# DJATOM/x265-aMod

Measured on AMD Instinct MI355X. Metric: encoded frames/sec at 1080p & 2160p --preset medium; bit-exact vs CPU ref, higher is better.
Workload: dtype u8

## Files before the change

include/x265amd.h:

```cpp
#ifndef X265AMD_H
#define X265AMD_H

#include <stdint.h>
#include <stddef.h>

#ifdef __cplusplus
extern "C" {
#endif

#ifndef X265AMD_DEPTH
#define X265AMD_DEPTH 8
#endif
#if X265AMD_DEPTH > 8
typedef uint16_t x265amd_pixel;
#else
typedef uint8_t x265amd_pixel;
#endif

#define X265AMD_OK 0
#define X265AMD_EINVAL (-1)
#define X265AMD_EHIP (-2)
#define X265AMD_ENOMEM (-3)

int x265amd_bit_depth(void);
// ... 349 lines not shown
    int32_t stride[3];
    int32_t bitDepth;
    int32_t layout;
    int32_t clipMin, clipMax;
    int32_t reserved;
} x265amd_surface;
#endif
int x265amd_ingest_picture(void* stream, const x265amd_surface* d_src, int srcW, int srcH,
                           x265amd_pixel* d_pic , int W, int H, int marginX, int marginY);
int x265amd_ingest_model(const x265amd_surface* src, int srcW, int srcH, x265amd_pixel* pic, int W, int H, int marginX, int marginY);

#define X265AMD_DB_INTRA 1
#define X265AMD_DB_CBF 2
#define X265AMD_DB_BYPASS 4
#define X265AMD_DB_TU_LEFT 8
#define X265AMD_DB_PU_LEFT 16
#define X265AMD_DB_TU_TOP 32
#define X265AMD_DB_PU_TOP 64
typedef struct x265amd_slice_info x265amd_slice_info;
typedef struct x265amd_mvpred_info x265amd_mvpred_info;
typedef struct x265amd_cu_unit x265amd_cu_unit;
typedef struct x265amd_mv_unit x265amd_mv_unit;
typedef struct x265amd_deblock_unit { uint8_t flags; int8_t qp; int8_t ref[2]; int16_t mv[2][2]; } x265amd_deblock_unit;
int x265amd_deblock_picture(void* stream, x265amd_pixel* d_y, x265amd_pixel* d_u, x265amd_pixel* d_v, intptr_t stride, intptr_t cstride,
                            int width, int height, const x265amd_deblock_unit* d_units, int betaOffsetDiv2, int tcOffsetDiv2,
                            int cbQpOffset, int crQpOffset, int bypassEnabled, int passes);

int x265amd_deblock_rows(void* stream, x265amd_pixel* d_y, x265amd_pixel* d_u, x265amd_pixel* d_v, intptr_t stride, intptr_t cstride,
                         int width, int height, const x265amd_deblock_unit* d_units, int betaOffsetDiv2, int tcOffsetDiv2,
                         int cbQpOffset, int crQpOffset, int bypassEnabled, int passes, int y4_begin, int y4_end);
int x265amd_deblock_rows_cols(void* stream, x265amd_pixel* d_y, x265amd_pixel* d_u, x265amd_pixel* d_v, intptr_t stride, intptr_t cstride,
                              int width, int height, const x265amd_deblock_unit* d_units, int betaOffsetDiv2, int tcOffsetDiv2,
                              int cbQpOffset, int crQpOffset, int bypassEnabled, int passes, int y4_begin, int y4_end, int ctu_col_begin, int ctu_col_end);

int x265amd_deblock_units(const x265amd_slice_info* si, const x265amd_mvpred_info* info, const x265amd_cu_unit* units, const x265amd_mv_unit* motion,
                          x265amd_deblock_unit* out);
int x265amd_deblock_units_rows(const x265amd_slice_info* si, const x265amd_mvpred_info* info, const x265amd_cu_unit* units, const x265amd_mv_unit* motion,
                               x265amd_deblock_unit* out, int y4_begin, int y4_end);
int x265amd_deblock_units_rect(const x265amd_slice_info* si, const x265amd_mvpred_info* info, const x265amd_cu_unit* units, const x265amd_mv_unit* motion,
                               x265amd_deblock_unit* out, int y4_begin, int y4_end, int x4_begin, int x4_end);

typedef struct x265amd_sao_ctu
{
    int8_t type[2];
    uint8_t band_pos[3];
    int8_t offset[3][4];
    uint8_t reserved[3];
} x265amd_sao_ctu;
int x265amd_sao_stats(void* stream, const uint64_t rec_planes[3], const uint64_t fenc_planes[3], intptr_t stride, intptr_t cstride,
                      int width, int height, int32_t* d_count, int32_t* d_offset_org);
int x265amd_sao_apply(void* stream, const uint64_t src_planes[3], const uint64_t dst_planes[3], intptr_t stride, intptr_t cstride,
                      int width, int height, const x265amd_sao_ctu* d_params);
int x265amd_sao_stats_rows(void* stream, const uint64_t rec_planes[3], const uint64_t fenc_planes[3], intptr_t stride, intptr_t cstride,
                           int width, int height, int32_t* d_count, int32_t* d_offset_org, int ctu_row_begin, int ctu_row_end);
int x265amd_sao_apply_rows(void* stream, const uint64_t src_planes[3], const uint64_t dst_planes[3], intptr_t stride, intptr_t cstride,
                           int width, int height, const x265amd_sao_ctu* d_params, int ctu_row_begin, int ctu_row_end);
int x265amd_sao_stats_rows_cols(void* stream, const uint64_t rec_planes[3], const uint64_t fenc_planes[3], intptr_t stride, intptr_t cstride,
                                int width, int height, int32_t* d_count, int32_t* d_offset_org, int ctu_row_begin, int ctu_row_end, int ctu_col_begin, int ctu_col_end);
int x265amd_sao_apply_rows_cols(void* stream, const uint64_t src_planes[3], const uint64_t dst_planes[3], intptr_t stride, intptr_t cstride,
                                int width, int height, const x265amd_sao_ctu* d_params, int ctu_row_begin, int ctu_row_end, int x_begin, int x_end);
enum { X265AMD_SAO_NON_DEBLOCK = 1, X265AMD_SAO_EO01_ONLY = 2 };
int x265amd_sao_stats_opt(void* stream, const uint64_t rec_planes[3], const uint64_t fenc_planes[3], intptr_t stride, intptr_t cstride,
                          int width, int height, int32_t* d_count, int32_t* d_offset_org, int flags);
int x265amd_sao_stats_opt_rows(void* stream, const uint64_t rec_planes[3], const uint64_t fenc_planes[3], intptr_t stride, intptr_t cstride,
                               int width, int height, int32_t* d_count, int32_t* d_offset_org, int flags, int ctu_row_begin, int ctu_row_end);
int x265amd_sao_stats_opt_rows_cols(void* stream, const uint64_t rec_planes[3], const uint64_t fenc_planes[3], intptr_t stride, intptr_t cstride,
                                    int width, int height, int32_t* d_count, int32_t* d_offset_org, int flags, int ctu_row_begin, int ctu_row_end, int ctu_col_begin, int ctu_col_end);
int x265amd_sao_stats_pre(void* stream, const uint64_t rec_planes[3], const uint64_t fenc_planes[3], intptr_t stride, intptr_t cstride,
                          int width, int height, int32_t* d_pre_count, int32_t* d_pre_offset_org);
int x265amd_sao_stats_pre_rows(void* stream, const uint64_t rec_planes[3], const uint64_t fenc_planes[3], intptr_t stride, intptr_t cstride,
                               int width, int height, int32_t* d_pre_count, int32_t* d_pre_offset_org, int ctu_row_begin, int ctu_row_end);
int x265amd_sao_stats_model(const void* const rec_planes[3], const void* const fenc_planes[3], const void* const pre_planes[3], intptr_t stride, intptr_t cstride,
                            int width, int height, int flags, int32_t* pre_count, int32_t* pre_offset_org, int32_t* count, int32_t* offset_org);

enum { X265AMD_FILTER_TOP = 0, X265AMD_FILTER_FULL = 1 };
typedef struct x265amd_filter_step { int32_t kind, row, col_begin, col_end, y4_begin, y4_end, rec_y4_end, rec_x4_begin, rec_x4_end; } x265amd_filter_step;
typedef struct x265amd_filter_finish { int32_t row, x_begin, x_end, y_begin, y_end; } x265amd_filter_finish;
int x265amd_filter_plan(int width, int height, const int32_t* analysed, int32_t* done_top, int32_t* done_full, int32_t* pub_x,
                        int min_chunk, int min_chunk_last, int early_top,
                        x265amd_filter_step* steps, int* num_steps, x265amd_filter_finish* finish, int* num_finish);
int x265amd_filter_ready(int width, int height, const int32_t* analysed, const int32_t* done_top, const int32_t* done_full,
                         int min_chunk, int min_chunk_last, int early_top);

enum { X265AMD_MODE_NONE = 0, X265AMD_MODE_INTER = 1, X265AMD_MODE_INTRA = 2, X265AMD_MODE_SKIP = 3 };
typedef struct x265amd_cu_unit
{
    uint8_t depth;
    uint8_t pred_mode;
    uint8_t part_size;
    uint8_t tu_depth;
    uint8_t luma_dir, chroma_dir;
    uint8_t merge_flag, inter_dir;
    uint8_t cbf[3];
    uint8_t tq_bypass;
    int8_t qp;
    int8_t ref_idx[2];
    uint8_t mvp_idx[2];
    uint8_t reserved;
    int16_t mvd[2][2];
} x265amd_cu_unit;
typedef struct x265amd_slice_info
{
    int32_t pic_width, pic_height;
    int32_t slice_type;
    int32_t slice_qp;
    int32_t num_ref_idx[2];
    int32_t max_num_merge_cand;
    int32_t use_dqp, max_cu_dqp_depth;
    int32_t sign_hide, tq_bypass_enabled;
    int32_t wpp;
    int32_t max_cu_depth;
    int32_t max_amp_depth;
    int32_t tu_log2_min, tu_log2_max;
    int32_t tu_max_depth_inter, tu_max_depth_intra;
} x265amd_slice_info;
#define X265AMD_SLICE_SIGN_HIDE 1
#define X265AMD_SLICE_LOWPASS_DCT 0x100
typedef struct x265amd_cabac x265amd_cabac;
x265amd_cabac* x265amd_cabac_open(const x265amd_slice_info* si, x265amd_cu_unit* units, int bits_only);
void x265amd_cabac_close(x265amd_cabac*);
void x265amd_cabac_set_contexts(x265amd_cabac*, const uint8_t* ctx);
void x265amd_cabac_get_contexts(const x265amd_cabac*, uint8_t* ctx);
int x265amd_cabac_encode_ctu(x265amd_cabac*, int ctu_addr, const int16_t* coeffY, const int16_t* coeffU, const int16_t* coeffV);
uint64_t x265amd_cabac_frac_bits(const x265amd_cabac*);
uint64_t x265amd_cabac_ctu_bits(const x265amd_cabac*);
size_t x265amd_cabac_finish_slice(x265amd_cabac*, uint8_t* out, size_t cap);

typedef struct x265amd_mv_unit { uint8_t pred_mode, inter_dir; int8_t ref_idx[2]; int16_t mv[2][2]; } x265amd_mv_unit;
typedef struct x265amd_mvpred_info
{
    int32_t pic_width, pic_height;
    int32_t is_inter_b, num_ref_idx[2], max_num_merge_cand;
    int32_t temporal_mvp;
    int32_t col_from_l0, check_ldc;
    int32_t poc, ref_poc[2][16];
    int32_t col_poc, col_ref_poc[2][16];
} x265amd_mvpred_info;
typedef struct x265amd_merge_cand { int16_t mv[2][2]; int8_t ref_idx[2]; uint8_t dir; uint8_t reserved; } x265amd_merge_cand;
int x265amd_merge_candidates(const x265amd_mvpred_info* info, const x265amd_mv_unit* cur, const x265amd_mv_unit* col, int cu_x, int cu_y, int log2_cu_size,
                             int part_size, int pu_idx, x265amd_merge_cand* out);
int x265amd_amvp_candidates(const x265amd_mvpred_info* info, const x265amd_mv_unit* cur, const x265amd_mv_unit* col, int cu_x, int cu_y, int log2_cu_size,
                            int part_size, int pu_idx, int list, int ref_idx, int16_t amvp[2][2], int16_t mvc[12][2]);

typedef struct x265amd_inter_search_params
{
    int32_t search_method, subpel_refine, search_range;
    int32_t qp;
    int32_t chroma_mc;
    int32_t ref_pic[2][16];
    int32_t frame_parallel;
    int32_t lazy_sync;
    int32_t lowres_blocks_in_row;
    int32_t me_pic[2][16];
    int32_t weighted;
    x265amd_weight wp[2][16][3];
    uint64_t lowres_mvs[2][16];
} x265amd_inter_search_params;
typedef struct x265amd_inter_cu { int16_t x, y; uint8_t log2_size, part_size; uint8_t reserved[2]; } x265amd_inter_cu;
typedef struct x265amd_pu_result
{
    uint8_t merge_flag, inter_dir;
    int8_t ref_idx[2];
    uint8_t mvp_idx[2];
    uint8_t reserved[2];
    int16_t mv[2][2], mvd[2][2];
} x265amd_pu_result;
// ... 298 lines not shown
```

x265-amod_amd/csrc/encoder_api.hip:

```cpp
#include "encoder_impl.h"
#include "ingest_dev.h"

extern "C" void x265amd_param_default(x265amd_param* p)
{
    if (!p) return;
    memset(p, 0, sizeof(*p));
    p->fpsNum = 25; p->fpsDenom = 1;
    p->bframes = 0; p->keyframeMax = 250; p->maxNumReferences = 3; p->qp = 30; p->ipFactor = 1.4f; p->pbFactor = 1.3f;
    p->rateControlMode = X265AMD_RC_CQP; p->rfConstant = 28; p->aqStrength = 1.0; p->qCompress = 0.6; p->aqMode = 0; p->cuTree = 0; p->qgSize = 32; p->qpMin = 0; p->qpMax = 69; p->vuiVideoFormat = 5; p->vuiColorPrimaries = 2; p->vuiTransfer = 2; p->vuiMatrix = 2; p->bEmitCLL = 1;
    p->rdLevel = 3; p->limitReferences = 3; p->bEnableEarlySkip = 1; p->recursionSkipMode = 1; p->bIntraInBFrames = 1; p->psyRd = 2.0; p->edgeVarThreshold = 0.05f;
    p->searchMethod = X265AMD_ME_HEX; p->subpelRefine = 2; p->searchRange = 57; p->maxNumMergeCand = 3;
    p->bEnableSignHiding = 1; p->bEnableStrongIntraSmoothing = 1; p->bEnableTemporalMvp = 1; p->tuQTMaxInterDepth = 1; p->tuQTMaxIntraDepth = 1;
    p->bEnableLoopFilter = 1; p->bEnableSAO = 1; p->bEnableWavefront = 1; p->aspectRatioIdc = 0;
}

void x265amd_encoder::fillStreamParams(x265amd_stream_params& s) const
{
    memset(&s, 0, sizeof(s));
    static const struct { uint32_t maxLumaSamples, maxLumaSamplesPerSecond; int idc; } levels[] = {
        { 36864, 552960, 30 }, { 122880, 3686400, 60 }, { 245760, 7372800, 63 }, { 552960, 16588800, 90 }, { 983040, 33177600, 93 },
        { 2228224, 66846720, 120 }, { 2228224, 133693440, 123 }, { 8912896, 267386880, 150 }, { 8912896, 534773760, 153 },
        { 8912896, 1069547520, 156 }, { 35651584, 1069547520, 180 }, { 35651584, 2139095040u, 183 }, { 35651584, 4278190080u, 186 } };
    s.profile_idc = X265AMD_DEPTH <= 8 ? 1 : 2;
    s.profile_compatibility_flags = X265AMD_DEPTH <= 8 ? (1u << 1) | (1u << 2) : (1u << 2);
// ... 248 lines not shown
    e->fillStreamParams(sp);
    e->headerBytes.resize(512);
    const size_t n = x265amd_write_stream_headers(&sp, e->headerBytes.data(), e->headerBytes.size());
    if (!n || n > e->headerBytes.size()) { xa_fail(X265AMD_EINVAL, "encoder_open: stream headers"); return nullptr; }
    e->headerBytes.resize(n);
    if (p->bEmitHDR10SEI || p->hasMasteringDisplay || p->maxCLL || p->maxFALL)
    {
        uint8_t sei[64], payload[24];
        if (p->bEmitCLL)
        {
            payload[0] = (uint8_t)(p->maxCLL >> 8); payload[1] = (uint8_t)p->maxCLL; payload[2] = (uint8_t)(p->maxFALL >> 8); payload[3] = (uint8_t)p->maxFALL;
            const size_t m = x265amd_write_sei(0, 144, payload, 4, sei, sizeof(sei));
            if (!m) { xa_fail(X265AMD_EINVAL, "encoder_open: content light level SEI"); return nullptr; }
            e->headerBytes.insert(e->headerBytes.end(), sei, sei + m);
        }
        if (p->hasMasteringDisplay)
        {
            for (int i = 0; i < 8; i++) { payload[2 * i] = (uint8_t)(p->masteringDisplay[i] >> 8); payload[2 * i + 1] = (uint8_t)p->masteringDisplay[i]; }
            for (int i = 0; i < 2; i++)
                for (int k = 0; k < 4; k++) payload[16 + 4 * i + k] = (uint8_t)(p->masteringDisplay[8 + i] >> (24 - 8 * k));
            const size_t m = x265amd_write_sei(0, 137, payload, 24, sei, sizeof(sei));
            if (!m) { xa_fail(X265AMD_EINVAL, "encoder_open: mastering display SEI"); return nullptr; }
            e->headerBytes.insert(e->headerBytes.end(), sei, sei + m);
        }
    }
    if (p->bEmitInfoSEI)
    {
        char text[1024];
        snprintf(text, sizeof(text), "x265amd (x265 build 209 interface) - %s - H.265/HEVC codec on AMD Instinct MI355X - options: %dx%d fps=%u/%u bitdepth=%d %s=%g aq-mode=%d aq-strength=%.2f "
                 "cutree=%d qcomp=%.2f qg-size=%d bframes=%d b-adapt=%d b-pyramid=%d open-gop=%d keyint=%d min-keyint=%d scenecut=%d rc-lookahead=%d lookahead-slices=%d ref=%d limit-refs=%d "
                 "rd=%d rdoq-level=%d psy-rd=%.2f me=%d subme=%d merange=%d max-merge=%d rect=%d amp=%d limit-modes=%d early-skip=%d rskip=%d weightp=%d weightb=%d sao=%d deblock=%d wpp=%d "
                 "tu-intra-depth=%d tu-inter-depth=%d signhide=%d strong-intra-smoothing=%d temporal-mvp=%d b-intra=%d fast-intra=%d sao-non-deblock=%d selective-sao=%d limit-sao=%d",
                 x265amd_version(), p->sourceWidth, p->sourceHeight, p->fpsNum, p->fpsDenom, X265AMD_DEPTH, p->rateControlMode == X265AMD_RC_CRF ? "crf" : "qp",
                 p->rateControlMode == X265AMD_RC_CRF ? p->rfConstant : (double)p->qp, e->aqOn ? p->aqMode : 0, p->aqStrength, p->cuTree != 0, p->qCompress, p->qgSize, p->bframes, p->bFrameAdaptive,
                 p->bBPyramid != 0, p->bOpenGOP != 0, p->keyframeMax, e->keyframeMin, p->scenecutThreshold, p->lookaheadDepth, p->lookaheadSlices, p->maxNumReferences, p->limitReferences,
                 p->rdLevel, p->rdoqLevel, p->psyRd, p->searchMethod, p->subpelRefine, p->searchRange, p->maxNumMergeCand, p->bEnableRectInter != 0, p->bEnableAMP != 0, p->limitModes != 0,
                 p->bEnableEarlySkip != 0, p->recursionSkipMode, p->bEnableWeightedPred != 0, p->bEnableWeightedBiPred != 0, p->bEnableSAO != 0, p->bEnableLoopFilter != 0, p->bEnableWavefront != 0,
                 p->tuQTMaxIntraDepth, p->tuQTMaxInterDepth, p->bEnableSignHiding != 0, p->bEnableStrongIntraSmoothing != 0, p->bEnableTemporalMvp != 0, p->bIntraInBFrames != 0, p->bEnableFastIntra != 0,
                 e->saoNonDeblock, e->selectiveSAO, e->limitSAO);
        if (e->lowPassDct) strncat(text, " lowpass-dct=1", sizeof(text) - strlen(text) - 1);
        uint8_t sei[1400];
        const size_t m = x265amd_write_info_sei(text, sei, sizeof(sei));
        if (!m) { xa_fail(X265AMD_EINVAL, "encoder_open: info SEI"); return nullptr; }
        e->headerBytes.insert(e->headerBytes.end(), sei, sei + m);
    }
    return e.release();
}

static PicP picByCoding(x265amd_encoder* e, uint64_t k)
{
    std::lock_guard<std::mutex> lk(e->byCodingMu);
    auto it = e->byCoding.find(k);
    return it == e->byCoding.end() ? PicP() : it->second;
}
static void rowRanges(const x265amd_encoder& e, int row, uint64_t off[3], uint64_t bytes[3])
{
    for (int k = 0; k < 3; k++)
    {
        const int sh = k ? 1 : 0, my = e.marginY >> sh, mx = e.marginX >> sh, h = e.H >> sh, rowH = 64 >> sh;
        const intptr_t st = k ? e.cstride : e.stride;
        const int y0 = row == 0 ? -my : row * rowH, y1 = row == e.ctuH - 1 ? h + my : std::min(h, (row + 1) * rowH);
        const int64_t first = (int64_t)e.org[k] + (int64_t)y0 * st - mx;
        off[k] = (uint64_t)first * sizeof(pixel);
        bytes[k] = (uint64_t)((int64_t)(y1 - y0) * st) * sizeof(pixel);
    }
}
extern "C" int x265amd_encoder_ctu_rows(const x265amd_encoder* e) { return e ? e->ctuH : -1; }
extern "C" int x265amd_encoder_stats(const x265amd_encoder* e, uint64_t* out, int n)
{
    if (!e || !out || n < 4) return xa_fail(X265AMD_EINVAL, "encoder_stats: arguments"), -1;
    out[0] = e->statPictures[0]; out[1] = e->statPictures[1]; out[2] = e->statPictures[2]; out[3] = e->statReferences;
    if (n >= 13)
        for (int t = 0; t < 3; t++) { out[4 + t] = e->statEmitted[t]; out[7 + t] = e->statBits[t]; memcpy(&out[10 + t], &e->statQpSum[t], 8); }
    if (n >= 31)
    {
        for (int g = 0; g < 4; g++)
        {
            for (int k = 0; k < 3; k++) memcpy(&out[13 + 4 * g + k], &e->statPsnr[g][k], 8);
            memcpy(&out[13 + 4 * g + 3], &e->statSsim[g], 8);
        }
        out[29] = e->statMaxCll;
        memcpy(&out[30], &e->statFallSum, 8);
    }
    return 0;
}
extern "C" int x265amd_encoder_quality(const x265amd_encoder* e, x265amd_quality* out)
{
    if (!e || !out) return xa_fail(X265AMD_EINVAL, "encoder_quality: arguments"), -1;
    if (!e->haveQuality || !e->lastQuality.measured) return -1;
    *out = e->lastQuality;
    return 0;
}
int x265amd_encoder::measureLevel(Pic& pic)
{
    x265amd_luma_level_record level;
    if (x265amd_luma_level(nullptr, planeAddr(pic.dSrc, 0), stride, srcW, srcH, levelDev) != X265AMD_OK) return -1;
    if (hipMemcpy(&level, levelDev, sizeof(level), hipMemcpyDeviceToHost) != hipSuccess) return xa_fail(X265AMD_EHIP, "encoder_encode: light level");
    x265amd_quality_values v;
    if (x265amd_quality_finish(nullptr, nullptr, &level, W, H, srcW, srcH, &v) != X265AMD_OK) return xa_fail(X265AMD_EINVAL, "encoder_encode: light level");
    pic.quality.lumaSum = level.sum; pic.quality.maxLumaLevel = level.max; pic.quality.avgLumaLevel = v.avgLumaLevel; pic.quality.measured |= 4;
    return 0;
}
extern "C" int x265amd_encoder_row_geometry(const x265amd_encoder* e, int row, x265amd_row_export* out)
{
    if (!e || !out || row < 0 || row >= e->ctuH) return xa_fail(X265AMD_EINVAL, "encoder_row_geometry: bad arguments"), -1;
    memset(out, 0, sizeof(*out));
    out->ctu_row = row;
    rowRanges(*e, row, out->plane_offset, out->plane_bytes);
    const size_t u0 = (size_t)row * 16 * e->w4, u1 = (size_t)std::min(e->h4, (row + 1) * 16) * e->w4;
    out->units_bytes = (u1 - u0) * sizeof(x265amd_cu_unit); out->map_offset_units = u0 * sizeof(x265amd_cu_unit);
    out->motion_bytes = (u1 - u0) * sizeof(x265amd_mv_unit); out->map_offset_motion = u0 * sizeof(x265amd_mv_unit);
    return 0;
}
extern "C" int x265amd_encoder_is_referenced(x265amd_encoder* e, uint64_t k)
{
    if (!e) return xa_fail(X265AMD_EINVAL, "encoder_is_referenced: null"), -1;
    PicP pic = picByCoding(e, k);
    if (!pic)
    {
        std::lock_guard<std::mutex> lk(e->byCodingMu);
        if (k < e->collectedCoding) return xa_fail(X265AMD_EINVAL, "encoder_is_referenced: that picture has been collected and released"), -1;
        return 2;
    }
    return pic->type != TYPE_B;
}
extern "C" int x265amd_encoder_owns(const x265amd_encoder* e, uint64_t k) { return e ? (e->p.shardCount <= 1 || (int)(k % (uint64_t)e->p.shardCount) == e->p.shardRank) : 0; }
extern "C" int x265amd_encoder_export_row(x265amd_encoder* e, uint64_t codingIndex, int row, x265amd_row_export* out, int timeoutMs)
{
    if (!e || !out || row < 0 || row >= e->ctuH) return xa_fail(X265AMD_EINVAL, "encoder_export_row: bad arguments"), -1;
    if (!e->frameParallel) return xa_fail(X265AMD_EINVAL, "encoder_export_row: rows are published by objects that code pictures in parallel (frameNumThreads > 1)"), -1;
    PicP pic = picByCoding(e, codingIndex);
    if (!pic)
    {
        std::lock_guard<std::mutex> lk(e->byCodingMu);
        if (codingIndex < e->collectedCoding) return xa_fail(X265AMD_EINVAL, "encoder_export_row: that picture has been collected and released: the pump is more than eight pictures late"), -1;
        return 1;
    }
    if (!pic->owned) return xa_fail(X265AMD_EINVAL, "encoder_export_row: this object does not code that picture"), -1;
    const auto t0 = std::chrono::steady_clock::now();
    while (pic->published(row) < e->W)
    {
        if (pic->failed.load()) return xa_fail(X265AMD_EHIP, "encoder_export_row: the picture failed"), -1;
        if (timeoutMs <= 0) return 2;
        if (std::chrono::duration<double, std::milli>(std::chrono::steady_clock::now() - t0).count() > timeoutMs) return xa_fail(X265AMD_EHIP, "encoder_export_row: time-out"), -1;
        std::this_thread::sleep_for(std::chrono::microseconds(200));
    }
    if (pic->failed.load()) return xa_fail(X265AMD_EHIP, "encoder_export_row: the picture failed"), -1;
    memset(out, 0, sizeof(*out));
    out->coding_index = codingIndex; out->ctu_row = row;
    rowRanges(*e, row, out->plane_offset, out->plane_bytes);
    for (int k = 0; k < 3; k++) out->src[k] = (const uint8_t*)pic->finalPlanes() + out->plane_offset[k];
    const size_t u0 = (size_t)row * 16 * e->w4, u1 = (size_t)std::min(e->h4, (row + 1) * 16) * e->w4;
    out->units = pic->units.data() + u0; out->units_bytes = (u1 - u0) * sizeof(x265amd_cu_unit); out->map_offset_units = u0 * sizeof(x265amd_cu_unit);
    out->motion = pic->motion.data() + u0; out->motion_bytes = (u1 - u0) * sizeof(x265amd_mv_unit); out->map_offset_motion = u0 * sizeof(x265amd_mv_unit);
    return 0;
}
extern "C" int x265amd_encoder_import_row(x265amd_encoder* e, const x265amd_row_export* in)
{
    if (!e || !in || in->ctu_row < 0 || in->ctu_row >= e->ctuH || !in->src[0] || !in->src[1] || !in->src[2] || !in->units || !in->motion) return xa_fail(X265AMD_EINVAL, "encoder_import_row: bad arguments"), -1;
    PicP pic = picByCoding(e, in->coding_index);
    if (!pic)
    {
        std::lock_guard<std::mutex> lk(e->byCodingMu);
        if (in->coding_index < e->collectedCoding) return xa_fail(X265AMD_EINVAL, "encoder_import_row: that picture has been collected and released"), -1;
        return 1;
    }
// ... 180 lines not shown
}
static int encoder_encode_impl(x265amd_encoder* e, x265amd_nal** ppNal, uint32_t* piNal, const x265amd_picture* picIn, x265amd_picture* picOut, bool inputOnDevice,
                               const x265amd_surface* surfIn)
{
    if (!e) return xa_fail(X265AMD_EINVAL, "encoder_encode: null encoder");
    if (ppNal) *ppNal = nullptr;
    if (piNal) *piNal = 0;
    const bool haveInput = picIn || surfIn;
    if (haveInput)
    {
        PicP pic(new Pic);
        pic->pool = e->laPool;
        pic->poc = e->frameCount++;
        const auto tu0 = std::chrono::steady_clock::now();
        int rc = surfIn ? e->ingestSurface(surfIn, *pic, inputOnDevice) : e->uploadPicture(picIn, *pic, inputOnDevice);
        if (rc) return -1;
        if (e->measuresLevel() && e->measureLevel(*pic)) return -1;
        const auto tl0 = std::chrono::steady_clock::now();
        e->uploadMs += std::chrono::duration<double, std::milli>(tl0 - tu0).count();
        if (e->lookahead && (rc = e->lowresInit(*pic)) != X265AMD_OK) return -1;
        e->laInitMs += std::chrono::duration<double, std::milli>(std::chrono::steady_clock::now() - tl0).count();
        e->input.push_back(pic);
    }
    const bool flushing = !haveInput;
    auto decide = [e, flushing]() -> int {
        const auto tl1 = std::chrono::steady_clock::now();
        int rc = X265AMD_OK;
        if (e->lookahead) rc = e->decideLookahead(flushing, flushing ? 1 : 1 << 30);
        else e->decideMiniGop(flushing);
        const double ms = std::chrono::duration<double, std::milli>(std::chrono::steady_clock::now() - tl1).count();
        e->laDecideMs += ms;
        static const bool timingD = xa_env_present("X265AMD_TIMING");
        if (timingD && ms > 0.5) fprintf(stderr, "x265amd: decision: %.1f ms, %d pictures typed, %d still in the lookahead%s\n", ms, (int)e->ready.size(), (int)e->input.size(), flushing ? " (flushing)" : "");
        return rc;
    };
    auto admit = [e]() -> int {
        while (!e->ready.empty())
        {
            PicP pic = e->ready.front();
            e->ready.pop_front();
            if (e->prepare(pic)) return -1;
            if (pic->dFin && !e->picSao(*pic))
            {
                if (hipStreamSynchronize(nullptr) != hipSuccess) return -1;
                xa_scratch_free(pic->dFin); pic->dFin = nullptr;
            }
            pic->codingOrder = e->codingCount++;
            pic->owned = e->p.shardCount <= 1 || (int)(pic->codingOrder % (uint64_t)e->p.shardCount) == e->p.shardRank;
            e->inflight.push_back(pic);
            { std::lock_guard<std::mutex> lk(e->byCodingMu); e->byCoding[pic->codingOrder] = pic; }
        }
        return 0;
    };
    if (decide() != X265AMD_OK || admit()) return -1;
    const bool timing = xa_env_present("X265AMD_TIMING");
    auto start = [e, timing](const PicP& pic) {
        std::shared_future<int> prev = e->lastTask;
        pic->started = true;
        if (timing) fprintf(stderr, "x265amd: poc %d handed to a frame task at %.1f ms (%d running)\n", pic->poc, Pic::pubClockMs(), e->running);
        pic->done = std::async(std::launch::async, [e, pic, prev, timing]() {
            xa_thread_device();
            const auto t0 = std::chrono::steady_clock::now();
            if (!pic->owned)
            {
                if (pic->type == TYPE_B) { if (!e->keepSources()) { xa_scratch_free(pic->dSrc); pic->dSrc = nullptr; } return (int)X265AMD_OK; }
                std::unique_lock<std::mutex> lk(pic->mu);
                static const int importWaitS = xa_env_int("X265AMD_IMPORT_WAIT_S", 300);
                const bool ok = pic->cv.wait_for(lk, std::chrono::seconds(importWaitS), [&] { return pic->importedRows >= e->ctuH || pic->failed.load(); });
                if (!ok || pic->failed.load()) { lk.unlock(); pic->fail(); return xa_fail(X265AMD_EHIP, "encoder: a picture coded elsewhere did not arrive"); }
                lk.unlock();
                if (!e->keepSources()) { xa_scratch_free(pic->dSrc); pic->dSrc = nullptr; }
                return (int)X265AMD_OK;
            }
            const int rc = e->frameParallel ? e->runFrameParallel(pic) : e->runFrame(pic, prev);
            { struct timespec ts; clock_gettime(CLOCK_THREAD_CPUTIME_ID, &ts); e->cpuPictureNs += (uint64_t)ts.tv_sec * 1000000000ull + (uint64_t)ts.tv_nsec; }
            if (timing)
                fprintf(stderr, "x265amd: poc %d type %d qp %d: %.2f ms\n", pic->poc, pic->type, pic->sliceQp,
                        std::chrono::duration<double, std::milli>(std::chrono::steady_clock::now() - t0).count());
            return rc;
        }).share();
        e->lastTask = pic->done;
        e->running++;
    };
    const int earlyPMax = 6;
    const int earlyBMax = e->ctuH > 24 ? 12 : 0;
    auto launch = [&]() {
    const bool headLong = !e->inflight.empty() && (e->inflight.front()->type == TYPE_IDR || e->inflight.front()->type == TYPE_I) && e->inflight.front()->started &&
                          e->inflight.front()->done.wait_for(std::chrono::seconds(0)) != std::future_status::ready;
    for (auto& q : e->inflight)
    {
        if (q->started) continue;
        if (e->running <= e->frameThreads || q == e->inflight.front()) { start(q); if (e->frameThreads <= 1) q->done.wait(); continue; }
        if (!e->frameParallel) break;
        if (q->type == TYPE_IDR || q->type == TYPE_I) start(q);
        else if (headLong && q->type == TYPE_P && e->running <= e->frameThreads + earlyPMax) start(q);
        else if (earlyBMax > 0 && headLong && e->running <= e->frameThreads + earlyBMax) start(q);
    }
    };
    launch();
    while (flushing && !e->input.empty())
    {
        if (!e->inflight.empty() && e->inflight.front()->started && e->inflight.front()->done.wait_for(std::chrono::seconds(0)) == std::future_status::ready) break;
        const size_t before = e->input.size();
        if (decide() != X265AMD_OK || admit()) return -1;
        launch();
        if (e->input.size() >= before) break;
    }
    if (e->inflight.empty()) return 0;
    PicP front = e->inflight.front();
    if (!front->started) { xa_fail(X265AMD_EINVAL, "encoder_encode: the first picture in coding order has no task"); return -1; }
    int waiting = 0;
    for (auto& q : e->inflight) waiting += !q->started;
    const bool mustWait = !haveInput || (e->running > e->frameThreads && waiting > 2 * e->p.lookaheadDepth + 8);
    if (!mustWait && front->done.wait_for(std::chrono::seconds(0)) != std::future_status::ready) return 0;
    const int rc = front->done.get();
    e->inflight.pop_front();
    e->running--;
    {
        std::lock_guard<std::mutex> lk(e->byCodingMu);
        e->collectedCoding = front->codingOrder + 1;
        while (!e->byCoding.empty() && e->byCoding.begin()->first + 8 < e->collectedCoding) e->byCoding.erase(e->byCoding.begin());
    }
    if (rc) { xa_fail(rc, "encoder_encode: a frame task failed"); return -1; }
    if (const char* dumpPath = xa_env_str("X265AMD_RC_DUMP"))
    {
        if (FILE* f = fopen(dumpPath, "ab"))
        {
            const Pic& q = *front;
            const int blocks16 = ((e->W + 15) / 16) * ((e->H + 15) / 16), lowresBlocks = e->lowCuW * e->lowCuH;
            int32_t hdr[44];
            memset(hdr, 0, sizeof(hdr));
            hdr[0] = 0x52434450; hdr[1] = q.poc; hdr[2] = q.type; hdr[3] = q.type != TYPE_B; hdr[4] = q.sliceQp; hdr[5] = q.bScenecut;
            for (int l = 0; l < 2; l++) { hdr[6 + l] = (int32_t)q.lists[l].size(); for (size_t r = 0; r < q.lists[l].size() && r < 16; r++) hdr[8 + 16 * l + r] = q.lists[l][r]->poc; }
            hdr[40] = e->w4; hdr[41] = e->h4; hdr[42] = blocks16; hdr[43] = lowresBlocks;
            fwrite(hdr, sizeof(hdr), 1, f);
            const int64_t satd = 0; fwrite(&satd, 8, 1, f);
            const double qq[2] = { q.avgQpRc, 0 }; fwrite(qq, 8, 2, f);
            std::vector<double> zd((size_t)blocks16, 0.0); std::vector<int32_t> zi((size_t)std::max(blocks16, lowresBlocks), 0); std::vector<uint16_t> zs((size_t)lowresBlocks, 0);
            fwrite(q.qpAqOffset.size() == (size_t)blocks16 ? q.qpAqOffset.data() : zd.data(), 8, blocks16, f);
            fwrite(q.qpCuTreeOffset.size() == (size_t)blocks16 ? q.qpCuTreeOffset.data() : zd.data(), 8, blocks16, f);
            fwrite(q.invQscale.size() == (size_t)blocks16 ? q.invQscale.data() : zi.data(), 4, blocks16, f);
            fwrite(q.intraCostHost.size() == (size_t)lowresBlocks ? q.intraCostHost.data() : zi.data(), 4, lowresBlocks, f);
            fwrite(q.propagateCost.size() == (size_t)lowresBlocks ? q.propagateCost.data() : zs.data(), 2, lowresBlocks, f);
            const size_t n = (size_t)e->w4 * e->h4;
            std::vector<uint8_t> b(n);
            for (size_t i = 0; i < n; i++) b[i] = (uint8_t)q.units[i].qp; fwrite(b.data(), 1, n, f);
            for (size_t i = 0; i < n; i++) b[i] = q.units[i].depth; fwrite(b.data(), 1, n, f);
            for (size_t i = 0; i < n; i++) b[i] = q.units[i].pred_mode; fwrite(b.data(), 1, n, f);
            for (size_t i = 0; i < n; i++) b[i] = q.units[i].cbf[0]; fwrite(b.data(), 1, n, f);
            fclose(f);
        }
    }
    e->outBytes.swap(front->nalBytes);
    const bool withAud = e->p.bEnableAccessUnitDelimiters && (front->poc || e->p.bRepeatHeaders) && !e->outBytes.empty();
    const bool withHeaders = e->p.bRepeatHeaders && front->bKeyframe && !e->outBytes.empty();
    if (withAud || withHeaders)
    {
        std::vector<uint8_t> au;
        if (withAud)
        {
            uint8_t aud[16];
            const size_t m = x265amd_write_aud(isBType(front->type) ? 0 : front->type == TYPE_P ? 1 : 2, aud, sizeof(aud));
            au.insert(au.end(), aud, aud + m);
        }
        if (withHeaders) au.insert(au.end(), e->headerBytes.begin(), e->headerBytes.end());
        const std::vector<uint8_t>& b = e->outBytes;
        for (size_t i = 0; i < b.size(); i++)
        {
            if (i + 4 <= b.size() && !b[i] && !b[i + 1] && !b[i + 2] && b[i + 3] == 1) continue;
            au.push_back(b[i]);
        }
        e->outBytes.swap(au);
    }
    bool haveStaging = false;
    if (e->p.decodedPictureHashSEI && !e->outBytes.empty())
    {
        e->staging.resize(e->picElems);
        if (hipMemcpy(e->staging.data(), front->finalPlanes(), e->picElems * sizeof(pixel), hipMemcpyDeviceToHost) != hipSuccess) { xa_fail(X265AMD_EHIP, "encoder: recon download"); return -1; }
        haveStaging = true;
        const void* planes[3] = { e->staging.data() + e->org[0], e->staging.data() + e->org[1], e->staging.data() + e->org[2] };
        const intptr_t strides[3] = { (intptr_t)(e->stride * sizeof(pixel)), (intptr_t)(e->cstride * sizeof(pixel)), (intptr_t)(e->cstride * sizeof(pixel)) };
        uint8_t payload[64], sei[96];
        const size_t n = x265amd_picture_hash(e->p.decodedPictureHashSEI, planes, strides, e->W, e->H, X265AMD_DEPTH, 64, payload, sizeof(payload));
        const size_t m = n ? x265amd_write_sei(1, 132, payload, n, sei, sizeof(sei)) : 0;
        if (!m) { xa_fail(X265AMD_EINVAL, "encoder: picture hash SEI"); return -1; }
        e->outBytes.insert(e->outBytes.end(), sei, sei + m);
    }
    splitNals(e->outBytes, e->nals);
// ... 41 lines not shown
```

x265-amod_amd/csrc/encoder_impl.h:

```cpp
#ifndef X265AMD_ENCODER_IMPL_H
#define X265AMD_ENCODER_IMPL_H
#include <hip/hip_runtime.h>
#include "x265amd.h"
#include "x265amd_encoder.h"
#include "x265amd_host.h"
#include "x265amd_ratecontrol.h"
#include <immintrin.h>
#include "xa_fiber.h"
#include <limits.h>
#include <math.h>
#include <stdio.h>
#include <stdlib.h>
#include <chrono>
#include <string.h>
#include <algorithm>
#include <atomic>
#include <condition_variable>
#include <deque>
#include <map>
#include <mutex>
#include <thread>
#include <future>
#include <memory>
#include <vector>
// ... 64 lines not shown
    std::vector<int32_t> lowMvc[18], lowMvc1[18];
    int64_t cost2[18][18];
    std::vector<int16_t> specMvs[18], specMvs1[18];
    std::vector<int32_t> specMvc[18], specMvc1[18];
    int64_t specCost2[18][18]; int specIntraMbs[18];
    uint64_t wpSum[3] = { 0, 0, 0 }, wpSsd[3] = { 0, 0, 0 };
    int lumaDenom = 7, chromaDenom = 7;
    x265amd_weight wp[2][16][3];
    bool weighted = false;
    bool bScenecut = false, bKeyframe = false;
    std::vector<int8_t> tuRecs;
    std::unique_ptr<x265amd_hist_scene_pic> hist;
    bool bHistScenecutAnalyzed = false;
    x265amd_quality quality;
    uint32_t* edgeCounts = nullptr;
    std::vector<int32_t> intraCostHost;
    std::vector<double> qpAqOffset, qpCuTreeOffset;
    std::vector<int32_t> invQscale;
    std::vector<uint16_t> propagateCost;
    std::map<int, void*> dLc, dSpecLc;
    std::map<int, std::vector<uint16_t> > lcHost;
    std::shared_ptr<LaPool> pool;
    void dropLc(std::map<int, void*>& m, int key) { auto it = m.find(key); if (it != m.end()) { if (pool) pool->put(it->second); m.erase(it); } }
    double avgQpRc = 0;
    bool bLastMiniGopBFrame = false;
    std::vector<int8_t> cuQp;
    const x265amd_mv_unit* regMotion = nullptr;
    void registerMotion()
    {
        if (regMotion == motion.data()) return;
        if (regMotion) xa_devmap_unregister(regMotion);
        regMotion = motion.data();
        if (!xa_devmap_register(regMotion, motion.size())) regMotion = nullptr;
    }
    Pic() { memset(refPoc, 0, sizeof(refPoc)); memset(wp, 0, sizeof(wp)); memset(&quality, 0, sizeof(quality)); for (int i = 0; i < 18; i++) { costEst[i] = -1; intraMbs[i] = 0; specIntraMbs[i] = 0; for (int j = 0; j < 18; j++) cost2[i][j] = specCost2[i][j] = -1; } }
    ~Pic() { if (pool) { for (auto& e : dLc) pool->put(e.second); for (auto& e : dSpecLc) pool->put(e.second);
                         for (int i = 0; i < 18; i++) for (const std::vector<int16_t>* v : { &lowMvs[i], &lowMvs1[i], &specMvs[i], &specMvs1[i] }) if (!v->empty()) pool->dead(v->data()); } if (regMotion) xa_devmap_unregister(regMotion); xa_scratch_free(dSrc); xa_scratch_free(dRec); xa_scratch_free(dFin); xa_scratch_free(dLowres); xa_scratch_free(dIntraCost); if (edgeCounts) xa_mapped_free(edgeCounts); for (volatile uint64_t* c : finalX) xa_counter_free(c); }
    void publish(int row, int x)
    {
        std::atomic_thread_fence(std::memory_order_release); *finalX[row] = (uint64_t)x;
        static const bool pubLog = xa_env_present("X265AMD_PUB_LOG");
        if (pubLog) fprintf(stderr, "x265amd pub: poc %d row %d x %d at %.2f\n", poc, row, x, pubClockMs());
    }
    static double pubClockMs() { return fmod(std::chrono::duration<double, std::milli>(std::chrono::steady_clock::now().time_since_epoch()).count(), 1e6); }
    int published(int row) const { const int v = (int)*finalX[row]; std::atomic_thread_fence(std::memory_order_acquire); return v; }
    void fail()
    {
        failed.store(true, std::memory_order_release);
        for (volatile uint64_t* c : finalX) *c = 1u << 30;
        { std::lock_guard<std::mutex> lk(mu); }
        cv.notify_all();
    }
};

}
using namespace xaenc;

struct x265amd_encoder
{
    x265amd_param p;
    x265amd_me_ctx* me = nullptr;
    int W = 0, H = 0, w4 = 0, h4 = 0, ctuW = 0, ctuH = 0, nctu = 0;
    int srcW = 0, srcH = 0;
    int marginX = 96, marginY = 80;
    intptr_t stride = 0, cstride = 0;
    size_t org[3] = { 0, 0, 0 }, picElems = 0;
    int qpConstant[3] = { 0, 0, 0 };
    int maxDecPicBuffering = 0, numReorderPics = 0;
    int frameCount = 0, lastKeyframe = 0, lastIDR = 0;
    bool haveKeyframe = false, refreshPending = false;
    int pocCRA = 0;
    bool first = true;
    std::deque<PicP> input;
    std::deque<PicP> ready;
    std::deque<PicP> inflight;
    uint64_t codingCount = 0;
    int running = 0;
    std::mutex importMu;
    hipStream_t importStream = nullptr;
    std::mutex byCodingMu;
    std::map<uint64_t, PicP> byCoding;
    uint64_t collectedCoding = 0;
    uint64_t statPictures[3] = { 0, 0, 0 }, statReferences = 0;
    uint64_t statEmitted[3] = { 0, 0, 0 }, statBits[3] = { 0, 0, 0 }; double statQpSum[3] = { 0, 0, 0 };
    double statPsnr[4][3] = { { 0, 0, 0 }, { 0, 0, 0 }, { 0, 0, 0 }, { 0, 0, 0 } }, statSsim[4] = { 0, 0, 0, 0 }, statFallSum = 0;
    uint32_t statMaxCll = 0;
    x265amd_quality lastQuality = {}; bool haveQuality = false;
    x265amd_luma_level_record* levelDev = nullptr;
    bool measuresLevel() const { return (p.maxCLL || p.maxFALL) && p.shardCount <= 1; }
    int measureLevel(Pic& pic);
    int measureQuality(Pic& pic, hipStream_t st);
    std::shared_future<int> lastTask;
    int frameThreads = 1;
    double uploadMs = 0;
    std::atomic<uint64_t> cpuPictureNs{ 0 }, cpuFilterNs{ 0 };
    bool frameParallel = false;
    int refLagRows = 0;
    std::vector<PicP> picList;
    double depthSaoRate[8] = { 0, 0, 0, 0, 0, 0, 0, 0 };
    std::vector<uint8_t> headerBytes, outBytes;
    std::vector<x265amd_nal> nals;
    std::vector<pixel> staging;
    pixel* uploadBuf = nullptr;
    int selectiveSAO = 0; bool limitSAO = false, saoNonDeblock = false;
    bool lowPassDct = false;
    bool picSao(const Pic& pic) const
    {
        if (!p.bEnableSAO) return false;
        const bool sliceI = pic.type == TYPE_IDR || pic.type == TYPE_I;
        if (selectiveSAO == 1) return sliceI;
        if (selectiveSAO == 2) return !(p.bframes != 0 && isBType(pic.type));
        if (selectiveSAO == 3) return pic.type != TYPE_B;
        return true;
    }
    int saoStatFlags(const Pic& pic) const { return (saoNonDeblock ? X265AMD_SAO_NON_DEBLOCK : 0) | (limitSAO && isBType(pic.type) ? X265AMD_SAO_EO01_ONLY : 0); }
    int32_t* dSaoPreCount = nullptr; int32_t* dSaoPreOrg = nullptr;
    int32_t* dSaoCount = nullptr; int32_t* dSaoOrg = nullptr; x265amd_sao_ctu* dSaoParams = nullptr; x265amd_deblock_unit* dDbUnits = nullptr;
    pixel* dSaoTmp = nullptr;

    ~x265amd_encoder()
    {
        for (auto& q : inflight) if (q->done.valid()) q->done.wait();
        laFieldsFree();
        if (uploadBuf) (void)hipHostFree(uploadBuf);
        if (ingestPinned) (void)hipHostFree(ingestPinned);
        if (xa_env_present("X265AMD_TIMING") && lookahead)
        {
            fprintf(stderr, "x265amd: input: %.1f ms in uploads; cpu of the picture threads %.1f ms, of the filter threads %.1f ms\n", uploadMs, cpuPictureNs.load() / 1e6, cpuFilterNs.load() / 1e6);
            fprintf(stderr, "x265amd: lookahead: %.1f ms in lowres planes + intra costs, %.1f ms in the slice-type decision (%llu estimates, %llu motion searches; %llu batches %.1f ms, %llu single estimates %.1f ms)\n", laInitMs, laDecideMs,
                    (unsigned long long)laJobs, (unsigned long long)laSearches, (unsigned long long)laBatches, laBatchMs, (unsigned long long)laSingles, laSingleMs);
            fprintf(stderr, "x265amd: lookahead estimates by phase: set-up %.1f ms, launch call %.1f, read-back issued %.1f, waited for %.1f, host sums %.1f; %llu weight guesses measured\n", laPhaseMs[0], laPhaseMs[1], laPhaseMs[2], laPhaseMs[3], laPhaseMs[4], (unsigned long long)laWeightJobs);
        }
        if (me) x265amd_me_close(me);
        if (rateCtl) x265amd_rc_close(rateCtl);
        if (dSaoPreCount) (void)hipFree(dSaoPreCount);
        if (dSaoPreOrg) (void)hipFree(dSaoPreOrg);
        if (dSaoCount) (void)hipFree(dSaoCount);
        if (dSaoOrg) (void)hipFree(dSaoOrg);
        if (dSaoParams) (void)hipFree(dSaoParams);
        if (dDbUnits) (void)hipFree(dDbUnits);
        xa_scratch_free(dSaoTmp);
        xa_scratch_free(histRecord);
        xa_scratch_free(levelDev);
        if (histRecordHost) xa_mapped_free(histRecordHost);
        if (laStream) (void)hipStreamDestroy(laStream);
        if (importStream) (void)hipStreamDestroy(importStream);
    }
    uint64_t planeAddr(const pixel* base, int k) const { return (uint64_t)(uintptr_t)(base + org[k]); }

    void fillStreamParams(x265amd_stream_params& s) const;
    int uploadPicture(const x265amd_picture* in, Pic& pic, bool onDevice = false);
    int ingestSurface(const x265amd_surface* in, Pic& pic, bool onDevice);
    uint8_t* ingestPinned = nullptr; size_t ingestPinnedBytes = 0;
    void decideMiniGop(bool flush);
    int prepare(const PicP& pic);
    int runFrame(const PicP& pic, std::shared_future<int> prev);
    int runFrameParallel(const PicP& pic);
    int edgeCounts(Pic& pic, hipStream_t st, x265amd_rskip_edge& edge);
    bool lookahead = false;
    void* wpEnergy = nullptr; void* wpSums = nullptr; void* wpSumsHost = nullptr; void* wpMvs = nullptr;
    int laRowsPerSlice = 0, laNumSlices = 1;
    int keyframeMin = 1, lowW = 0, lowH = 0, lowCuW = 0, lowCuH = 0, lowBlocks = 0;
    intptr_t lowStride = 0; size_t lowPlaneElems = 0, lowOrg = 0;
    PicP lastNonB;
    bool isSceneTransition = false;
    hipStream_t laStream = nullptr;
// ... 51 lines not shown
```

Baseline: 87.97.

## Plan frame task launches with reference-aware ahead-start rule

Moves the rule for starting frame tasks early into a separate planning function. While a long intra picture is still running, it starts referenced pictures first (cap raised from 6 to 12) and only when their references are already started, then fills leaf B pictures up to their own cap. The aim is more frame-level overlap without launching tasks that would stall on references that have not started. Launching more tasks ahead adds concurrency pressure and can cause contention; new counters track how many ahead starts happen.

New measurement: 96.41 (median of 6 runs). 1.1x the previous value.

```diff
diff --git a/include/x265amd.h b/include/x265amd.h
--- a/include/x265amd.h
+++ b/include/x265amd.h
@@ -455,6 +455,13 @@
 int x265amd_filter_ready(int width, int height, const int32_t* analysed, const int32_t* done_top, const int32_t* done_full,
                          int min_chunk, int min_chunk_last, int early_top);
 
+enum { X265AMD_LAUNCH_MAX_REFS = 32 };
+enum { X265AMD_LAUNCH_IN_TURN = 0, X265AMD_LAUNCH_INTRA = 1, X265AMD_LAUNCH_AHEAD_REF = 2, X265AMD_LAUNCH_AHEAD_LEAF = 3 };
+typedef struct x265amd_launch_pic { int32_t type, referenced, started, finished, num_refs; int32_t refs[X265AMD_LAUNCH_MAX_REFS]; } x265amd_launch_pic;
+int x265amd_launch_plan(const x265amd_launch_pic* pics, int num_pics, int running, int frame_threads, int ctu_h, int frame_parallel,
+                        int32_t* start, int32_t* ahead, int* num_start);
+int x265amd_launch_caps(int ctu_h, int* ref_cap, int* leaf_cap);
+
 enum { X265AMD_MODE_NONE = 0, X265AMD_MODE_INTER = 1, X265AMD_MODE_INTRA = 2, X265AMD_MODE_SKIP = 3 };
 typedef struct x265amd_cu_unit
 {
diff --git a/x265-amod_amd/csrc/encoder_api.hip b/x265-amod_amd/csrc/encoder_api.hip
--- a/x265-amod_amd/csrc/encoder_api.hip
+++ b/x265-amod_amd/csrc/encoder_api.hip
@@ -354,6 +354,7 @@
         out[29] = e->statMaxCll;
         memcpy(&out[30], &e->statFallSum, 8);
     }
+    if (n >= 33) { out[31] = e->statAheadRef; out[32] = e->statAheadLeaf; }
     return 0;
 }
 extern "C" int x265amd_encoder_quality(const x265amd_encoder* e, x265amd_quality* out)
@@ -700,28 +701,47 @@
         e->lastTask = pic->done;
         e->running++;
     };
-    const int earlyPMax = 6;
-    const int earlyBMax = e->ctuH > 24 ? 12 : 0;
-    auto launch = [&]() {
-    const bool headLong = !e->inflight.empty() && (e->inflight.front()->type == TYPE_IDR || e->inflight.front()->type == TYPE_I) && e->inflight.front()->started &&
-                          e->inflight.front()->done.wait_for(std::chrono::seconds(0)) != std::future_status::ready;
-    for (auto& q : e->inflight)
-    {
-        if (q->started) continue;
-        if (e->running <= e->frameThreads || q == e->inflight.front()) { start(q); if (e->frameThreads <= 1) q->done.wait(); continue; }
-        if (!e->frameParallel) break;
-        if (q->type == TYPE_IDR || q->type == TYPE_I) start(q);
-        else if (headLong && q->type == TYPE_P && e->running <= e->frameThreads + earlyPMax) start(q);
-        else if (earlyBMax > 0 && headLong && e->running <= e->frameThreads + earlyBMax) start(q);
-    }
+    auto launch = [&]() -> int {
+        const int n = (int)e->inflight.size();
+        if (!n) return 0;
+        std::vector<x265amd_launch_pic> plan((size_t)n);
+        std::vector<int32_t> order((size_t)n), how((size_t)n);
+        for (int i = 0; i < n; i++)
+        {
+            const Pic& q = *e->inflight[i];
+            x265amd_launch_pic& r = plan[i];
+            memset(&r, 0, sizeof(r));
+            r.type = q.type; r.referenced = q.type != TYPE_B; r.started = q.started;
+            r.finished = q.started && q.done.wait_for(std::chrono::seconds(0)) == std::future_status::ready;
+            const uint64_t first = e->inflight.front()->codingOrder;
+            for (int l = 0; l < 2; l++)
+                for (const PicP& ref : q.lists[l])
+                {
+                    const int at = ref->codingOrder >= first && ref->codingOrder < q.codingOrder && ref->codingOrder - first < (uint64_t)n &&
+                                   e->inflight[ref->codingOrder - first] == ref ? (int)(ref->codingOrder - first) : -1;
+                    bool seen = at < 0;
+                    for (int k = 0; k < r.num_refs && !seen; k++) seen = r.refs[k] == at;
+                    if (!seen && r.num_refs < X265AMD_LAUNCH_MAX_REFS) r.refs[r.num_refs++] = at;
+                }
+        }
+        int count = 0;
+        if (x265amd_launch_plan(plan.data(), n, e->running, e->frameThreads, e->ctuH, e->frameParallel, order.data(), how.data(), &count) != X265AMD_OK)
+            return xa_fail(X265AMD_EINVAL, "encoder_encode: the start rule refused the pictures in flight"), -1;
+        for (int k = 0; k < count; k++)
+        {
+            const PicP& q = e->inflight[order[k]];
+            start(q);
+            e->statAheadRef += how[k] == X265AMD_LAUNCH_AHEAD_REF; e->statAheadLeaf += how[k] == X265AMD_LAUNCH_AHEAD_LEAF;
+            if (e->frameThreads <= 1) q->done.wait();
+        }
+        return 0;
     };
-    launch();
+    if (launch()) return -1;
     while (flushing && !e->input.empty())
     {
         if (!e->inflight.empty() && e->inflight.front()->started && e->inflight.front()->done.wait_for(std::chrono::seconds(0)) == std::future_status::ready) break;
         const size_t before = e->input.size();
-        if (decide() != X265AMD_OK || admit()) return -1;
-        launch();
+        if (decide() != X265AMD_OK || admit() || launch()) return -1;
         if (e->input.size() >= before) break;
     }
     if (e->inflight.empty()) return 0;
diff --git a/x265-amod_amd/csrc/encoder_impl.h b/x265-amod_amd/csrc/encoder_impl.h
--- a/x265-amod_amd/csrc/encoder_impl.h
+++ b/x265-amod_amd/csrc/encoder_impl.h
@@ -170,6 +170,7 @@
     std::map<uint64_t, PicP> byCoding;
     uint64_t collectedCoding = 0;
     uint64_t statPictures[3] = { 0, 0, 0 }, statReferences = 0;
+    uint64_t statAheadRef = 0, statAheadLeaf = 0;
     uint64_t statEmitted[3] = { 0, 0, 0 }, statBits[3] = { 0, 0, 0 }; double statQpSum[3] = { 0, 0, 0 };
     double statPsnr[4][3] = { { 0, 0, 0 }, { 0, 0, 0 }, { 0, 0, 0 }, { 0, 0, 0 } }, statSsim[4] = { 0, 0, 0, 0 }, statFallSum = 0;
     uint32_t statMaxCll = 0;
diff --git a/x265-amod_amd/host/launch_plan.cpp b/x265-amod_amd/host/launch_plan.cpp
--- /dev/null
+++ b/x265-amod_amd/host/launch_plan.cpp
@@ -0,0 +1,67 @@
+#include "x265amd.h"
+
+namespace {
+
+inline bool isIntra(int t) { return t == 1 || t == 2; }
+
+const int kRefCap = 12;
+inline int leafCapOf(int ctuH) { return ctuH > 24 ? 12 : 0; }
+
+}
+
+extern "C" int x265amd_launch_caps(int ctu_h, int* ref_cap, int* leaf_cap)
+{
+    if (ctu_h <= 0 || !ref_cap || !leaf_cap) return X265AMD_EINVAL;
+    *ref_cap = kRefCap; *leaf_cap = leafCapOf(ctu_h);
+    return X265AMD_OK;
+}
+
+extern "C" int x265amd_launch_plan(const x265amd_launch_pic* pics, int num_pics, int running, int frame_threads, int ctu_h, int frame_parallel,
+                                   int32_t* start, int32_t* ahead, int* num_start)
+{
+    if (num_pics < 0 || (num_pics && !pics) || running < 0 || frame_threads < 1 || ctu_h <= 0 || !start || !num_start) return X265AMD_EINVAL;
+    for (int i = 0; i < num_pics; i++)
+    {
+        if (pics[i].num_refs < 0 || pics[i].num_refs > X265AMD_LAUNCH_MAX_REFS) return X265AMD_EINVAL;
+        for (int k = 0; k < pics[i].num_refs; k++)
+            if (pics[i].refs[k] < -1 || pics[i].refs[k] >= i) return X265AMD_EINVAL;
+    }
+    int n = 0;
+    *num_start = 0;
+    if (!num_pics) return X265AMD_OK;
+    auto startedAt = [&](int i) {
+        if (pics[i].started) return true;
+        for (int k = 0; k < n; k++) if (start[k] == i) return true;
+        return false;
+    };
+    auto refsStarted = [&](int i) {
+        for (int k = 0; k < pics[i].num_refs; k++)
+            if (pics[i].refs[k] >= 0 && !startedAt(pics[i].refs[k])) return false;
+        return true;
+    };
+    auto take = [&](int i, int how) { start[n] = i; if (ahead) ahead[n] = how; n++; running++; };
+
+    int next = 0;
+    for (; next < num_pics; next++)
+    {
+        if (pics[next].started) continue;
+        if (running <= frame_threads || next == 0) take(next, X265AMD_LAUNCH_IN_TURN);
+        else break;
+    }
+    if (frame_parallel && next < num_pics)
+    {
+        const bool headLong = isIntra(pics[0].type) && startedAt(0) && !pics[0].finished;
+        int refCap = 0, leafCap = 0;
+        if (headLong) { refCap = kRefCap; leafCap = leafCapOf(ctu_h); }
+        for (int i = next; i < num_pics; i++)
+        {
+            if (startedAt(i)) continue;
+            if (isIntra(pics[i].type)) take(i, X265AMD_LAUNCH_INTRA);
+            else if (pics[i].referenced && running <= frame_threads + refCap && refCap > 0 && refsStarted(i)) take(i, X265AMD_LAUNCH_AHEAD_REF);
+        }
+        for (int i = next; i < num_pics && leafCap > 0; i++)
+            if (!startedAt(i) && !pics[i].referenced && !isIntra(pics[i].type) && running <= frame_threads + leafCap && refsStarted(i)) take(i, X265AMD_LAUNCH_AHEAD_LEAF);
+    }
+    *num_start = n;
+    return X265AMD_OK;
+}
```
